# nktoan/h-edit

Hardware: AMD Instinct MI355X
Metric: edited images/sec (512^2, 50 steps, K Langevin) (higher is better)
Workload: dtype bf16

## Files before the change

h-edit_amd/build.py:

```python
#!/usr/bin/env python3
import os
import subprocess
import sys
from concurrent.futures import ThreadPoolExecutor

HERE = os.path.dirname(os.path.abspath(__file__))
SRC = os.path.join(HERE, "csrc")
OBJ = os.path.join(HERE, "build")
OUT = os.path.join(HERE, "hedit", "libhedit_hip.so")
UNITS = ["gemm.hip", "pgemm.hip", "pconv.hip", "ffn.hip", "linchain.hip", "norm.hip", "attn.hip", "attnbwd.hip", "step.hip", "grad.hip", "s2dgrad.hip", "pnet.hip", "encoder.hip", "store.hip", "unet.hip", "vae.hip", "ddpm.hip", "irse.hip", "faceparse.hip", "lpips.hip", "vit.hip", "text.hip", "clipimg.hip", "sqlpips.hip", "dino.hip", "pixmetrics.hip", "c_api.hip"]
FLAGS = ["--offload-arch=gfx950", "-O3", "-std=c++17", "-fPIC", "-ffp-contract=off", "-Wno-unused-result"]
UNIT_FLAGS = {"attn.hip": ["-fno-honor-nans"], "ffn.hip": ["-fno-honor-nans"]}


def _deps_mtime():
    hdrs = [os.path.join(SRC, f) for f in os.listdir(SRC) if f.endswith(".h")]
    hdrs.append(os.path.join(os.path.dirname(HERE), "include", "hedit.h"))
    return max(os.path.getmtime(p) for p in hdrs)


def build(force=False, verbose=True, f16=False):
    hipcc = os.environ.get("HIPCC", "/opt/rocm/bin/hipcc")
    OBJ = os.path.join(HERE, "build_f16" if f16 else "build")
    OUT = os.path.join(HERE, "hedit", "libhedit_hip_f16.so" if f16 else "libhedit_hip.so")
    FLAGS = globals()["FLAGS"] + (["-DHEDIT_STORE_F16"] if f16 else [])
    os.makedirs(OBJ, exist_ok=True)
    hm = _deps_mtime()
    jobs = []
    for u in UNITS:
        src = os.path.join(SRC, u)
        obj = os.path.join(OBJ, u.replace(".hip", ".o"))
        if force or not os.path.exists(obj) or os.path.getmtime(obj) < max(os.path.getmtime(src), hm):
            jobs.append((src, obj))

    def cc(job):
        src, obj = job
        cmd = [hipcc] + FLAGS + UNIT_FLAGS.get(os.path.basename(src), []) + ["-c", src, "-o", obj]
        r = subprocess.run(cmd, capture_output=True, text=True)
        if r.returncode != 0:
            raise RuntimeError(f"hipcc failed for {src}:\n{r.stderr[-4000:]}")
        return src

    if jobs:
        with ThreadPoolExecutor(max_workers=min(6, len(jobs))) as ex:
            for s in ex.map(cc, jobs):
                if verbose:
                    print("compiled", os.path.relpath(s, HERE))
    objs = [os.path.join(OBJ, u.replace(".hip", ".o")) for u in UNITS]
    if jobs or not os.path.exists(OUT):
        cmd = [hipcc, "--offload-arch=gfx950", "-shared", "-fPIC", "-o", OUT] + objs
        r = subprocess.run(cmd, capture_output=True, text=True)
        if r.returncode != 0:
            raise RuntimeError(f"link failed:\n{r.stderr[-4000:]}")
        if verbose:
            print("linked", os.path.relpath(OUT, HERE))
    return OUT


if __name__ == "__main__":
    build(force="--force" in sys.argv, f16="--f16" in sys.argv)
```

h-edit_amd/csrc/gemm.hip:

```cpp
#include <type_traits>

#include "common.h"
#include "gnstat.h"
#include "kernels.h"

namespace {

typedef __attribute__((ext_vector_type(4))) unsigned u32x4;
constexpr int BM0 = 128;
constexpr int BK = 64;

template <int BM, int BN, bool DEEP = false>
struct Smem {
  static constexpr int A_BYTES = BM * BK * 2;
  static constexpr int W_BYTES = BN * BK * 2;
  static constexpr int STAGE = A_BYTES + W_BYTES;
  static constexpr int STAGES = (DEEP || (BM == 256 && BN <= 160)) ? 3 : 2;
  static constexpr int EPI = BM * (BN + 8) * 2;
  static constexpr int TOTAL = STAGES * STAGE > EPI ? STAGES * STAGE : EPI;
  static constexpr int RS_W0 = 2 * A_BYTES;
  static constexpr int RS_ZERO = RS_W0 + 3 * W_BYTES;
  static constexpr int RS_TOTAL = RS_ZERO + A_BYTES + 128;
};

// ... 672 lines not shown
      float2* red = reinterpret_cast<float2*>(smem + RED_OFF);
      const int r = tid / CHUNKS, c = tid - r * CHUNKS;
      GnPiece t[2];
#pragma unroll
      for (int it = 0; it < ITER; ++it) {
        const GnPiece g = gns_piece(ov[it][0], ov[it][1], ov[it][2], ov[it][3]);
        if (gns_first<RSTEP>(it)) t[gns_slot<RSTEP>(it)] = g; else gns_add(t[gns_slot<RSTEP>(it)], g);
      }
      gns_store_t(red, gns_red_row<RSTEP>(r, 0), c, t[0]);
      gns_store_t(red, gns_red_row<RSTEP>(r, 1), c, t[1]);
      __syncthreads();
      if (tid < UNITS * 64) {
        const int u = tid >> 6, pk = tid & 63;
        const float2 v = gns_fold_unit(red, u, pk);
        if (m0 + u * GNS_UNIT < p.M)
          *reinterpret_cast<float2*>(p.gn_part + (((long)(m0 / GNS_UNIT + u) * (p.N / 2)) + n0 / 2 + pk) * 2) = v;
      }
    }
  } else {
    for (int idx = tid; idx < BM * CHUNKS * 2; idx += NT) {
      const int ml = idx / (CHUNKS * 2), h = idx - ml * (CHUNKS * 2);
      const int m = m0 + ml, n = n0 + h * 4;
      if (m >= p.M || n >= p.N) continue;
      uint2 o = *reinterpret_cast<const uint2*>(sc + ml * CS + h * 4);
      if (p.residual) {
        const uint2 r = *reinterpret_cast<const uint2*>(p.residual + (long)m * p.ldr + n);
        o.x = add2(o.x, r.x);
        o.y = add2(o.y, r.y);
      }
      *reinterpret_cast<uint2*>(p.C + (long)m * p.ldc + n) = o;
    }
  }
}

__global__ __launch_bounds__(256) void splitk_reduce_kernel(GemmParams p) {
  const long idx = (long)blockIdx.x * 256 + threadIdx.x;
  const int n4 = p.N / 4;
  const long total = (long)p.M * n4;
  if (idx >= total) return;
  const int m = (int)(idx / n4);
  const int n = (int)(idx - (long)m * n4) * 4;
  f32x4 v = {0.f, 0.f, 0.f, 0.f};
  for (int s = 0; s < p.splits; ++s)
    v += *reinterpret_cast<const f32x4*>(p.partial + ((long)s * p.M + m) * p.N + n);
  if (p.raw_f32) {
    *reinterpret_cast<f32x4*>(p.raw_f32 + (long)m * p.N + n) = v;
    return;
  }
  f32x4 b = {0.f, 0.f, 0.f, 0.f};
  if (p.bias) b = *reinterpret_cast<const f32x4*>(p.bias + n);
  v = v + b;
  uint2 o;
  o.x = pack_bf16x2(v[0], v[1]);
  o.y = pack_bf16x2(v[2], v[3]);
  if (p.residual) {
    const uint2 r = *reinterpret_cast<const uint2*>(p.residual + (long)m * p.ldr + n);
    o.x = pack_bf16x2(bf16_to_f32((bf16_t)(o.x & 0xffff)) + bf16_to_f32((bf16_t)(r.x & 0xffff)),
                      bf16_to_f32((bf16_t)(o.x >> 16)) + bf16_to_f32((bf16_t)(r.x >> 16)));
    o.y = pack_bf16x2(bf16_to_f32((bf16_t)(o.y & 0xffff)) + bf16_to_f32((bf16_t)(r.y & 0xffff)),
                      bf16_to_f32((bf16_t)(o.y >> 16)) + bf16_to_f32((bf16_t)(r.y >> 16)));
  }
  *reinterpret_cast<uint2*>(p.C + (long)m * p.ldc + n) = o;
}

__global__ __launch_bounds__(256) void splitk_reduce_gn_kernel(GemmParams p) {
  __shared__ float2 red[32 * 64];
  const int tid = threadIdx.x, r = tid >> 4, c = tid & 15;
  const int m0 = blockIdx.x * GNS_UNIT, n = blockIdx.y * 128 + c * 8;
  f32x4 b0 = {0.f, 0.f, 0.f, 0.f}, b1 = b0;
  if (p.bias) {
    b0 = *reinterpret_cast<const f32x4*>(p.bias + n);
    b1 = *reinterpret_cast<const f32x4*>(p.bias + n + 4);
  }
  auto add2 = [](uint32_t a, uint32_t b) __attribute__((always_inline)) {
    return pack_bf16x2(bf16_to_f32((bf16_t)(a & 0xffff)) + bf16_to_f32((bf16_t)(b & 0xffff)),
                       bf16_to_f32((bf16_t)(a >> 16)) + bf16_to_f32((bf16_t)(b >> 16)));
  };
  GnPiece t[2];
#pragma unroll
  for (int it = 0; it < 8; ++it) {
    const int m = m0 + r + 16 * it;
    f32x4 v0 = {0.f, 0.f, 0.f, 0.f}, v1 = v0;
    for (int s = 0; s < p.splits; ++s) {
      const float* src = p.partial + ((long)s * p.M + m) * p.N + n;
      v0 += *reinterpret_cast<const f32x4*>(src);
      v1 += *reinterpret_cast<const f32x4*>(src + 4);
    }
    v0 = v0 + b0;
    v1 = v1 + b1;
    u32x4 o = {pack_bf16x2(v0[0], v0[1]), pack_bf16x2(v0[2], v0[3]), pack_bf16x2(v1[0], v1[1]), pack_bf16x2(v1[2], v1[3])};
    if (p.residual) {
      const u32x4 rr = *reinterpret_cast<const u32x4*>(p.residual + (long)m * p.ldr + n);
      o[0] = add2(o[0], rr[0]); o[1] = add2(o[1], rr[1]); o[2] = add2(o[2], rr[2]); o[3] = add2(o[3], rr[3]);
    }
    *reinterpret_cast<u32x4*>(p.C + (long)m * p.ldc + n) = o;
    const GnPiece g = gns_piece(o[0], o[1], o[2], o[3]);
    if (gns_first<16>(it)) t[gns_slot<16>(it)] = g; else gns_add(t[gns_slot<16>(it)], g);
  }
  gns_store_t(red, gns_red_row<16>(r, 0), c, t[0]);
  gns_store_t(red, gns_red_row<16>(r, 1), c, t[1]);
  __syncthreads();
  if (tid < 64) {
    const float2 v = gns_fold_unit(red, 0, tid);
    *reinterpret_cast<float2*>(p.gn_part + ((long)blockIdx.x * (p.N / 2) + blockIdx.y * 64 + tid) * 2) = v;
  }
}

template <int BM, int BN, int MODE, bool CHUNK, bool DEEP = false>
int launch_igemm_impl(const GemmParams& p, int splits, hipStream_t st) {
  using S = Smem<BM, BN, DEEP>;
  constexpr int LDS = (MODE == 4 || MODE == 5) ? S::RS_TOTAL : S::TOTAL;
  dim3 grid(cdiv(p.M, BM) * cdiv(p.N, BN), splits);
#if HEDIT_F16
  if (p.op_bf16) {
    if (int rc = hedit_dyn_lds(reinterpret_cast<const void*>(&igemm_kernel<BM, BN, MODE, CHUNK, false, DEEP, false, true>), LDS)) return rc;
    hipLaunchKernelGGL((igemm_kernel<BM, BN, MODE, CHUNK, false, DEEP, false, true>), grid, dim3(BM * 2), LDS, st, p);
    LAUNCH_CHECK();
    return HEDIT_OK;
  }
#endif
  if constexpr (BN == 128 && MODE != 0) {
    if (p.gn_part && !p.partial) {
      if (int rc = hedit_dyn_lds(reinterpret_cast<const void*>(&igemm_kernel<BM, BN, MODE, CHUNK, false, DEEP, true>), LDS)) return rc;
      hipLaunchKernelGGL((igemm_kernel<BM, BN, MODE, CHUNK, false, DEEP, true>), grid, dim3(BM * 2), LDS, st, p);
      LAUNCH_CHECK();
      return HEDIT_OK;
    }
  }
  constexpr bool COUNTED = MODE == 4 || MODE == 5 || S::STAGES == 3;
  if constexpr (COUNTED) {
    if (hedit_test_drained()) {
      if (int rc = hedit_dyn_lds(reinterpret_cast<const void*>(&igemm_kernel<BM, BN, MODE, CHUNK, true, DEEP>), LDS)) return rc;
      hipLaunchKernelGGL((igemm_kernel<BM, BN, MODE, CHUNK, true, DEEP>), grid, dim3(BM * 2), LDS, st, p);
      LAUNCH_CHECK();
      return HEDIT_OK;
    }
  }
  if (int rc = hedit_dyn_lds(reinterpret_cast<const void*>(&igemm_kernel<BM, BN, MODE, CHUNK, false, DEEP>), LDS)) return rc;
  hipLaunchKernelGGL((igemm_kernel<BM, BN, MODE, CHUNK, false, DEEP>), grid, dim3(BM * 2), LDS, st, p);
  LAUNCH_CHECK();
  return HEDIT_OK;
}


template <int BN, int MODE>
int launch_igemm(const GemmParams& p, int splits, hipStream_t st) {
  const long tiles256 = (long)cdiv(p.M, 256) * cdiv(p.N, BN);
  const bool big = splits == 1 && (p.geglu || p.K / BK >= 16) && tiles256 >= 200;
  const bool chunk = splits == 1 && p.chunk_kt > 0 && p.chunk_kt < p.K / BK;
  if constexpr (MODE == 1) {
    if (big && splits == 1 && p.Hout == p.Hin && p.Wout == p.Win && p.Win > 0 && 256 % p.Win == 0) {
      if (!chunk) return launch_igemm_impl<256, BN, 4, false>(p, splits, st);
      if constexpr (BN == 128) return launch_igemm_impl<256, BN, 4, true>(p, splits, st);
    }
  }
  if constexpr (MODE == 3) {
    if (big && splits == 1 && p.Wout > 0 && 256 % p.Wout == 0) {
      if (!chunk) return launch_igemm_impl<256, BN, 5, false>(p, splits, st);
      if constexpr (BN == 128) return launch_igemm_impl<256, BN, 5, true>(p, splits, st);
    }
  }
  if (chunk)
    return big ? launch_igemm_impl<256, BN, MODE, true>(p, splits, st) : launch_igemm_impl<128, BN, MODE, true>(p, splits, st);
  if (big) return launch_igemm_impl<256, BN, MODE, false>(p, splits, st);
  int cus = 256;
  if (int rc = hedit_cu_count(&cus)) return rc;
  const long blocks = (long)cdiv(p.M, 128) * cdiv(p.N, BN) * splits;
  if (blocks <= cus && p.K / BK >= 3) return launch_igemm_impl<128, BN, MODE, false, true>(p, splits, st);
  return launch_igemm_impl<128, BN, MODE, false>(p, splits, st);
}

}

int gemm_pick_bn(int N);
static int pick_bn(const GemmParams& p) {
  if (p.geglu) return (p.N % 256 == 0 && (long)cdiv(p.M, 256) * (p.N / 256) >= 200) ? 256 : 128;
  return gemm_pick_bn(p.N);
}

int gemm_pick_bn(int N) {
  long w160 = (long)cdiv(N, 160) * 160, w128 = (long)cdiv(N, 128) * 128;
  return w160 <= w128 ? 160 : 128;
}

int gemm_canonical_chunk(int M_nom, int N_nom, int K) {
  const int bn = gemm_pick_bn(N_nom);
  const long tiles = (long)cdiv(M_nom, BM0) * cdiv(N_nom, bn);
  const int kt = K / BK;
  if (tiles >= 256 || kt < 24) return 0;
  int s = (int)((256 + tiles - 1) / tiles);
  int max_s = kt / 4;
  if (s > max_s) s = max_s;
  if (s > 16) s = 16;
  if (s <= 1) return 0;
  const int chunk = cdiv(kt, s);
  return chunk >= kt ? 0 : chunk;
}

int gemm_plan_splits(int M, int N, int K, int chunk_kt) {
  const int kt = K / BK;
  if (chunk_kt <= 0 || chunk_kt >= kt) return 1;
  const int s = cdiv(kt, chunk_kt);
  const long tiles = (long)cdiv(M, BM0) * cdiv(N, gemm_pick_bn(N));
  return tiles * s <= 1024 ? s : 1;
}

int gemm_pick_splits(int M, int N, int K, int force) {
  (void)M; (void)N;
  const int kt = K / BK;
  if (force <= 1) return 1;
  return force > kt ? kt : force;
}

size_t gemm_partial_bytes(int M, int N, int splits) {
  return splits > 1 ? (size_t)splits * M * N * sizeof(float) : 0;
}

static const bf16_t* zero_page_device() {
  static bf16_t* z = nullptr;
  if (!z) {
    void* ptr = nullptr;
    if (hipMalloc(&ptr, 256) != hipSuccess) return nullptr;
    if (hipMemset(ptr, 0, 256) != hipSuccess) return nullptr;
    z = reinterpret_cast<bf16_t*>(ptr);
  }
  return z;
}

int gemm_prepare() { return zero_page_device() ? HEDIT_OK : HEDIT_ERR_HIP; }

int gemm_launch(GemmParams p, int splits, float* partial_ws, hipStream_t st) {
  p.zeros = zero_page_device();
  if (!p.zeros) {
    hedit_set_error("gemm: could not allocate the zero page");
    return HEDIT_ERR_HIP;
  }
  ARG_CHECK(p.K % BK == 0, "gemm: K must be a multiple of 64");
  ARG_CHECK(p.N % 4 == 0, "gemm: N must be a multiple of 4");
  ARG_CHECK(p.mode >= 0 && p.mode <= 3, "gemm: mode");
  if (p.mode != 0) ARG_CHECK(p.Cin % BK == 0 && p.K == 9 * p.Cin, "gemm: conv needs Cin % 64 == 0 and K = 9 Cin");
  ARG_CHECK(p.ldc % 4 == 0 && (p.residual == nullptr || p.ldr % 4 == 0), "gemm: ldc/ldr alignment");
  {
    const double a_b = p.mode == 0 ? (double)p.M * p.lda * 2.0
                                   : (double)(p.M / ((long)p.Hout * p.Wout)) * p.Hin * p.Win * p.Cin * 2.0;
    const double w_b = (double)p.N * p.K * 2.0;
    ARG_CHECK(a_b < 2040.0 * 1048576.0 && w_b < 2040.0 * 1048576.0, "gemm: operand larger than 2 GiB");
    p.a_bytes = (unsigned)a_b;
    p.w_bytes = (unsigned)w_b;
  }
  const int kt = p.K / BK;
  if (splits < 1) splits = 1;
  if (splits > kt) splits = kt;
  if (p.chunk_kt < 0 || p.chunk_kt >= kt) p.chunk_kt = 0;
  if (splits > 1) {
    p.kt_per_split = p.chunk_kt > 0 ? p.chunk_kt : cdiv(kt, splits);
    p.splits = cdiv(kt, p.kt_per_split);
    ARG_CHECK(p.chunk_kt == 0 || p.splits == splits, "gemm: split count does not match the canonical chunking");
  } else {
    p.splits = 1;
    p.kt_per_split = kt;
  }
  splits = p.splits;
  if (p.raw_f32 && splits == 1) {
    ARG_CHECK(!p.geglu, "gemm: raw fp32 output excludes the GEGLU epilogue");
    p.partial = p.raw_f32;
  } else if (splits > 1) {
    ARG_CHECK(!p.geglu, "gemm: split-K excludes the GEGLU epilogue");
    ARG_CHECK(partial_ws != nullptr, "gemm: split-K needs a partial workspace");
    p.partial = partial_ws;
  } else {
    p.partial = nullptr;
  }
  ARG_CHECK(!p.op_bf16 || (p.raw_f32 && !p.geglu && !p.gn_part), "gemm: bfloat16-by-contract operands come with the raw fp32 output");
  if (p.gn_part) {
    ARG_CHECK(p.mode != 0 && !p.geglu && !p.raw_f32 && !p.ln_out, "gemm: pair statistics come with the bf16 tile of a convolution");
    ARG_CHECK(p.M % GNS_UNIT == 0 && p.N % 128 == 0 && gemm_pick_bn(p.N) == 128, "gemm: pair statistics need M % 128 == 0 and the 128-column tile");
    ARG_CHECK(p.ldc % 8 == 0 && (p.residual == nullptr || p.ldr % 8 == 0), "gemm: pair statistics need 16-byte rows");
  }
  int bn = pick_bn(p);
  if (splits == 1 && p.chunk_kt > 0 && p.mode == 3) bn = 128;
  if (splits == 1 && p.chunk_kt > 0 && p.mode == 1 && p.Hout == p.Hin && p.Wout == p.Win && p.Win > 0 && 256 % p.Win == 0 &&
      p.N % 128 == 0 && (long)cdiv(p.M, 256) * (p.N / 128) >= 512)
    bn = 128;
  if (p.geglu) {
    ARG_CHECK(p.N % 32 == 0 && p.mode == 0 && p.residual == nullptr && p.ldc % 8 == 0, "gemm: geglu epilogue needs N % 32 == 0, linear mode, no residual");
    ARG_CHECK(splits == 1 && p.chunk_kt == 0, "gemm: the geglu epilogue takes no K-chunking");
  }
  {
    const double a_bytes = (double)p.M * (p.mode == 0 ? p.K : p.Cin);
    const double w_bytes = (double)p.N * p.K;
    p.n_fastest = a_bytes >= w_bytes ? 1 : 0;
  }
  if (pgemm_supported(p, splits, bn)) return pgemm_launch(p, bn, st);
  if (pconv_supported(p, splits, bn)) return pconv_launch(p, bn, st);
  int rc;
#define DISPATCH(BNV)                                                     \
  switch (p.mode) {                                                       \
    case 0: rc = launch_igemm<BNV, 0>(p, splits, st); break;              \
    case 1: rc = launch_igemm<BNV, 1>(p, splits, st); break;              \
    case 2: rc = launch_igemm<BNV, 2>(p, splits, st); break;              \
    default: rc = launch_igemm<BNV, 3>(p, splits, st); break;             \
  }
  if (bn == 256) {
    rc = launch_igemm_impl<256, 256, 0, false>(p, 1, st);
  } else if (bn == 160) { DISPATCH(160) } else { DISPATCH(128) }
#undef DISPATCH
  if (rc != HEDIT_OK) return rc;
  if (splits > 1) {
    if (p.ln_out && p.ln_done && !p.raw_f32 && p.ldc == p.N && splitk_reduce_ln_supported(p.N)) {
      *p.ln_done = 1;
      return splitk_reduce_ln_launch(p.partial, p.splits, p.bias, p.residual, p.ldr, p.C, p.ln_out, p.ln_gamma, p.ln_beta, p.M, p.N,
                                     p.ln_eps, st);
    }
    if (p.gn_part) {
      hipLaunchKernelGGL(splitk_reduce_gn_kernel, dim3(p.M / GNS_UNIT, p.N / 128), dim3(256), 0, st, p);
      LAUNCH_CHECK();
      return HEDIT_OK;
    }
    long total = (long)p.M * (p.N / 4);
    hipLaunchKernelGGL(splitk_reduce_kernel, dim3(cdiv(total, 256)), dim3(256), 0, st, p);
    LAUNCH_CHECK();
  }
  return HEDIT_OK;
}
```

h-edit_amd/csrc/kernels.h:

```cpp
#pragma once
#include "common.h"

struct GemmParams {
  const bf16_t* A;
  const bf16_t* W;
  int M, N, K;
  int lda;
  int mode;
  int Hin, Win, Cin, Hout, Wout;
  const float* bias;
  const bf16_t* residual;
  int ldr;
  bf16_t* C;
  int ldc;
  float* partial;
  int splits, kt_per_split;
  int n_fastest;
  const bf16_t* zeros;
  unsigned a_bytes, w_bytes;
  int geglu;
  int asym;
  float* raw_f32;
  int chunk_kt;
  const float *ln_gamma, *ln_beta;
  bf16_t* ln_out;
  float ln_eps;
  int* ln_done;
  float* gn_part;
  int op_bf16;
};
#ifndef GEMM_NOMINAL_BATCH
#define GEMM_NOMINAL_BATCH 4
#endif
int gemm_prepare();
int gemm_pick_bn(int N);
int gemm_pick_splits(int M, int N, int K, int force);
int gemm_canonical_chunk(int M_nom, int N_nom, int K);
int gemm_plan_splits(int M, int N, int K, int chunk_kt);
size_t gemm_partial_bytes(int M, int N, int splits);
int gemm_launch(GemmParams p, int splits, float* partial_ws, hipStream_t st);
bool pgemm_supported(const GemmParams& p, int splits, int bn);
int pgemm_launch(const GemmParams& p, int bn, hipStream_t st);
bool pconv_supported(const GemmParams& p, int splits, int bn);
int pconv_launch(const GemmParams& p, int bn, hipStream_t st);

struct FfnParams {
  const bf16_t* x; long ldx;
  const float* gamma; const float* beta; float eps;
  const bf16_t* stream;
  const float* bias1p;
  const float* bias2;
  bf16_t* out; long ldo;
  int M, C;
  const bf16_t* a; long lda;
  const bf16_t* r2; long ldr2;
  const float* bias_pre; const float* bias_post;
};
struct LinChainParams {
  const bf16_t* a; long lda;
  const bf16_t* r1; long ldr1;
  const float* bias_pre;
  const float* gamma; const float* beta; float eps;
  const bf16_t* stream;
  bf16_t* out_mid; long ldmid;
  bf16_t* out; long ldo;
  int M, C;
  const float* gn_ss; int rows_per_image;
  bf16_t* out_q; long ldq; bf16_t* out_k; long ldk;
};
int lin_chain_launch(const LinChainParams& c, hipStream_t st);
int lin_chain_launch_sched(const LinChainParams& c, int sched, hipStream_t st);
size_t lin_chain_stream_bytes(int layers);
int lin_chain_pack_launch(const float* w, int layer, float scale, int layers, bf16_t* stream, hipStream_t st);
int ffn_fused_channels();
size_t ffn_stream_bytes(int pre, int post);
size_t ffn_bias_bytes();
int ffn_pack_launch(const float* w, int which, int pre, int post, bf16_t* stream, hipStream_t st);
int ffn_pack_bias_launch(const float* b1, float* out, hipStream_t st);
int ffn_fused_launch(const FfnParams& f, hipStream_t st);

#define HEDIT_MAXW 77
#define HEDIT_WPAD 96
#define HEDIT_CTXP 80

size_t groupnorm_ws_bytes(int B, int HW, int C);
int groupnorm_launch(const bf16_t* x, bf16_t* y, const float* gamma, const float* beta, int B,
                     int HW, int C, int G, float eps, int silu, float* ws, hipStream_t st,
                     float* stats = nullptr);
bool groupnorm_from_parts_supported(int HW, int C, int G);
size_t groupnorm_from_parts_ws_bytes(int B);
int groupnorm_from_parts_launch(const bf16_t* x, bf16_t* y, const float* gamma, const float* beta, int B, int HW, int C, int G,
                                float eps, int silu, const float* part_a, int ca, const float* part_b, int cb, float* ws,
                                hipStream_t st);
int groupnorm_affine_launch(const bf16_t* x, const float* gamma, const float* beta, int B, int HW, int C, int G, float eps,
                            float* ws, hipStream_t st, const float** ss_out);
int layernorm_launch(const bf16_t* x, bf16_t* y, const float* gamma, const float* beta, long rows,
                     int C, float eps, hipStream_t st);
bool splitk_reduce_ln_supported(int C);
int splitk_reduce_ln_launch(const float* partial, int splits, const float* bias, const bf16_t* residual, int ldr, bf16_t* out,
                            bf16_t* y, const float* gamma, const float* beta, long rows, int C, float eps, hipStream_t st);
int geglu_launch(const bf16_t* x, bf16_t* y, long rows, int inner, hipStream_t st);
#define HEDIT_ROWMAP_MAX 512
struct RowMap { uint16_t src[HEDIT_ROWMAP_MAX]; };
int concat_launch(const bf16_t* a, int ca, const bf16_t* b, int cb, bf16_t* y, long rows, hipStream_t st,
                  const RowMap* b_map = nullptr, int rows_per_image = 0);
int gather_rows_launch(const void* const* src, void* const* dst, int n, int B, long row_bytes, const RowMap& map, hipStream_t st);
int f32_to_bf16_launch(const float* x, bf16_t* y, long n, hipStream_t st);
int ctx_pad_launch(const float* x, bf16_t* y, int B, int dim, hipStream_t st);
int gemv_launch(const bf16_t* W, const float* x, const float* b0, const float* b1, float* out,
                int N, int K, int silu, hipStream_t st);
int copy_rows_launch(bf16_t* x, const int* src, int B, long row_elems, hipStream_t st);
int timestep_embed_launch(float t, float* out, int dim, hipStream_t st);
int timestep_embed_ddpm_launch(float t, float* out, int dim, hipStream_t st);
int conv_in_launch(const float* x, const float* w, const float* bias, bf16_t* y, int B, int Cin,
                   int H, int W, int Cout, hipStream_t st);
int conv_out_launch(const bf16_t* x, const bf16_t* w, const float* bias, float* y, int B, int H,
                    int W, int C, int Cout, hipStream_t st);
int rows_to_nchw_launch(const float* src, const float* bias, float* dst, int B, long HW, int ld, int Cout, hipStream_t st);
int softmax_rows_launch(const float* s, bf16_t* p, long rows, int N, float scale, hipStream_t st);
int softmax_blockdiag_launch(const float* s, bf16_t* p, long rows, int T, int ld, float scale, hipStream_t st);
int mix1x1_nchw_launch(const float* x, const float* w, const float* bias, float* y, int B, int Cin, int Cout, long HW,
                       float pre_scale, hipStream_t st);
int quant_mean_launch(const bf16_t* h, const float* w, const float* bias, float* y, int B, long HW, int Cm, int Cout, hipStream_t st);
int pack_linear_launch(const float* w, bf16_t* out, long n, float scale, hipStream_t st);
int pack_conv3x3_launch(const float* w_oihw, bf16_t* out, int O, int I, hipStream_t st);
int pack_geglu_rows_launch(const float* w, bf16_t* out_bf16, float* out_f32, int rows, int K, hipStream_t st);

size_t groupnorm_bwd_ws_bytes(int B, int HW, int C);
int groupnorm_bwd_launch(const bf16_t* x, const bf16_t* dy, const bf16_t* add, bf16_t* dx, const float* gamma,
                         const float* beta, const float* stats, int B, int HW, int C, int G, int silu, float* ws,
                         hipStream_t st, bool any_width = false);
int softmax_bwd_launch(const bf16_t* p, const float* dp, bf16_t* ds, long rows, int N, float scale, hipStream_t st);
int transpose_bf16_launch(const bf16_t* src, bf16_t* dst, int R, int C, hipStream_t st);
int sum2x2_launch(const bf16_t* du, bf16_t* dx, int B, int H, int W, int C, hipStream_t st);
int pack_conv3x3_dgrad_launch(const float* w_oihw, bf16_t* out, int O, int I, hipStream_t st);
int pack_linear_t_launch(const float* w, bf16_t* out, int O, int I, hipStream_t st, float scale = 1.f, long ldo = 0);
int flip_oihw_launch(const float* w, float* out, int O, int I, int k, hipStream_t st);
int layernorm_bwd_launch(const bf16_t* x, const bf16_t* dy, const bf16_t* add, bf16_t* dx, const float* gamma, long rows, int C,
                         float eps, hipStream_t st);
int geglu_bwd_launch(const bf16_t* x, const bf16_t* dy, bf16_t* dx, long rows, int inner, hipStream_t st);

int conv3x3_s2_dgrad_launch(const bf16_t* dy, const bf16_t* wt, bf16_t* dx, int B, int Hin, int Win, int O, int I, hipStream_t st);
int pack_conv3x3_s2_dgrad_launch(const float* w_oihw, bf16_t* out, int O, int I, hipStream_t st);
int conv3x3_s2_dgrad_pad1_launch(const bf16_t* dy, const bf16_t* wt, bf16_t* dx, int B, int Hin, int Win, int O, int I, hipStream_t st);
int slice_add_launch(const bf16_t* src, int ld, int off, int c, bf16_t* dst, long rows, int accumulate, hipStream_t st);

struct SelfAttnParams {
  const bf16_t* q; int ldq;
  const bf16_t* k; int ldk;
  const bf16_t* vt; long ldvt;
  bf16_t* out; int ldo;
  int B, N, heads, d;
  const int* qk_src;
  const int* kv_src;
  int test_flags;
};
int self_attn_launch(const SelfAttnParams& p, hipStream_t st);

struct CrossAttnParams {
  const bf16_t* q; int ldq;
  const bf16_t* k; int ldk;
  const bf16_t* vt; long ldvt;
  bf16_t* out; int ldo;
  int B, N, heads, d;
  int n_pairs;
  const int* pair_src;
  const int* pair_tar;
  const bf16_t* mixT;
  const float* bvec;
  float* store;
  const int* singles;
  int n_single;
};
int cross_attn_launch(const CrossAttnParams& p, hipStream_t st);

struct AttnProbsParams {
  const bf16_t* q; int ldq;
  const bf16_t* k; int ldk;
  const bf16_t* vt; long ldvt;
  float* probs;
  bf16_t* out; int ldo;
  int B, N, M, kstride, heads, d;
  const int *pair_src, *pair_tar, *qk_src;
};
int attn_probs_launch(const AttnProbsParams& p, hipStream_t st);
int attn_self_store_launch(const AttnProbsParams& p, hipStream_t st);
int attn_apply_launch(const AttnProbsParams& p, hipStream_t st);

struct AttnBwdParams {
  const bf16_t* q; int ldq;
  const bf16_t* k; int ldk;
  const bf16_t* v; int ldv;
  const bf16_t* o; int ldo;
  const bf16_t* dout; int lddo;
  bf16_t* dq; int lddq;
  bf16_t* dk; bf16_t* dv; int lddkv;
  float* stats;
  int B, N, M, kstride, heads, d;
};
size_t attn_bwd_ws_bytes(int B, int N, int heads);
int attn_bwd_launch(const AttnBwdParams& p, hipStream_t st);
int attn_bwd_ctx_chunk(int N);
size_t attn_bwd_ctx_kv_ws_bytes(int B, int N, int heads, int d);
int attn_bwd_ctx_kv_launch(const AttnBwdParams& p, float* part, hipStream_t st);

struct StepCoef {
  float sqrt_ab_t, sqrt_1m_ab_t;
  float sqrt_ab_prev;
  float dir_coef;
  float noise_coef;
  float w_src, w_hat, w_tar;
  float coeff;
  float w_rec;
};
int step_base_launch(const float* eps, const float* xt, const float* z, float* x_prev, int n_img,
                     int elems, int eps_rows_per_img, StepCoef c, hipStream_t st);
int step_pair_launch(const float* e_u, const float* e_c, const float* xt, const float* z, float* x_next, int n_img, int elems,
                     int n_kinds, const StepCoef* c, hipStream_t st);
int step_invert_launch(const float* e_u, const float* e_c, const float* xt, float* x_prev, float* z_out, int n_img,
                       int elems, StepCoef c, hipStream_t st);
int step_update_launch(const float* e_u_src, const float* e_c_src, const float* e_u_tar,
                       const float* e_c_tar, long stride_img, const float* x_k, const float* x_base,
                       float* x_out, int n_img, int elems, int k_gt0, StepCoef c, hipStream_t st);
int step_tweedie_launch(const float* e_u_tar, const float* e_c_tar, long stride_img, const float* x, float* z0,
                        int n_img, int elems, float w_tar, float sqrt_ab, float sqrt_1m_ab, float inv_scale, hipStream_t st);
int step_style_launch(const float* e_u_src, const float* e_c_src, const float* e_u_tar, const float* e_c_tar,
                      long stride_img, const float* x, const float* g_z, float* x_out, int n_img, int elems, float w_hat,
                      float w_tar, float chain, float weight, hipStream_t st);
int step_ef_seed_launch(const float* g_z, float* d_eps, int n_img, int elems, float w_tar, float c, hipStream_t st);
int step_ef_style_launch(const float* e_u, const float* e_c, long stride_img, const float* dx, const float* g_z,
                         const float* x_prev, float* x_out, int n_img, int elems, float a, float weight, hipStream_t st);
int axis_mix_launch(const float* in, float* out, const int* idx, const float* val, int nnz, long outer, int n_in, int n_out, int inner,
                    hipStream_t st);
int local_blend_launch(const float* const* maps, int n_maps, int heads, const float* alpha_layers, const float* alpha_sub,
                       const int* enabled, float* xt, int n_img, int C, int H, int W, float th, float th_sub, hipStream_t st);

enum { P_COPY = 0, P_AFFINE = 1, P_PRELU = 2, P_PRELU_GRAD = 3, P_RELU = 4, P_RELU_GRAD = 5, P_QGELU = 6, P_QGELU_GRAD = 7,
       P_AFFINE_RELU = 8,
       P_GELU = 9 };
struct Split3Params {
  const float* x; int ldx;
  const float* z;
  const float* p; const float* q;
  int pq_img;
  int op;
  bf16_t* out; int Kp, Cs, C;
  int geo;
  int B, H, W;
  int worder;
};
int split3_launch(const Split3Params& s, long rows_out, hipStream_t st);
int pack_split3_w_launch(const float* w, const float* scale, bf16_t* out, int O, int I, int k, int dgrad, int Cs, int Kp,
                         int rows_out, int perm_hw, int perm_c, hipStream_t st);
int bn_affine_launch(const float* g, const float* b, const float* m, const float* v, float eps, float* p, float* q, int C, int rep,
                     hipStream_t st);
int bn_fold_bias_launch(const float* bias, const float* g, const float* b, const float* m, const float* v, float eps, float* p, float* q,
                        int C, hipStream_t st);
int act_launch(const float* x, const float* p, const float* q, float* y, long total, int C, int op, hipStream_t st);
int se_nslab(int HW);
int se_pool_launch(const float* u, float* part, int B, int HW, int C, hipStream_t st);
int se_fc_launch(const float* part, const float* bias, const float* w1, const float* w2, float* hbuf, float* sbuf, int B, int HW, int C,
                 int R, hipStream_t st);
int se_combine_launch(const float* u, const float* bias, const float* s, const float* sc, const float* sc_bias, const float* X, int stride,
                      float* Y, int B, int Ho, int Wo, int C, hipStream_t st);
int se_bwd_reduce_launch(const float* dY, const float* u, const float* bias, float* part, int B, int HW, int C, hipStream_t st);
int se_fc_bwd_launch(const float* part, const float* sbuf, const float* hbuf, const float* w1, const float* w2, float* rbuf, int B, int C,
                     int R, int HW, hipStream_t st);
int unit_bwd_combine_launch(const float* dxa, const float* p, const float* dsc, int stride, float* dX, int B, int H, int W, int C,
                            hipStream_t st);
int scale_cols_launch(const float* x, const float* p, float* y, long total, int n, hipStream_t st);
int face_pool_launch(const float* img, float* out, int B, hipStream_t st);
int face_pool_bwd_launch(const float* g, int ldg, float* dimg, int B, hipStream_t st);
int cos_head_launch(const float* raw, const float* bias, const float* ref, int ref_stride, float* feat, float* loss, float* df, int B, int D,
                    float scale, hipStream_t st);
int lpips_prep_launch(const float* img, float* out, const float* shift3, const float* scale3, int B, int H, int W, hipStream_t st);
int lpips_prep_bwd_launch(const float* g, int ldg, float* dimg, const float* scale3, int B, int H, int W, hipStream_t st);
int maxpool2_launch(const float* z, float* zp, uint8_t* idx, int B, int H, int W, int C, hipStream_t st);
int maxpool2_bwd_launch(const float* gp, const uint8_t* idx, const float* add, float* G, int B, int H, int W, int C, hipStream_t st);
int lpips_head_launch(const float* z, const float* bias, const float* src, long src_img_stride, const float* w, float* fn_out, float* dpix,
                      float* dF, int B, int HW, int C, float gscale, hipStream_t st);
int lpips_reduce_launch(const float* dpix, float* acc, int B, int HW, int first, hipStream_t st);

int enc_patchify_launch(const float* img, float* X, int B, int R, int p, int bwd, hipStream_t st);
int enc_tokens_launch(const float* E, const float* cbias, const float* cls, const float* pos, float* T, int B, int L, int W, hipStream_t st);
int enc_gather_rows_launch(const float* T, const int32_t* idx, float* R, int B, int L, int W, hipStream_t st);
int enc_ln_launch(const float* x, const float* g, const float* b, float* y, float* stats, long rows, int W, float eps, hipStream_t st);
int enc_add_bias_res_launch(const float* raw, const float* bias, const float* res, float* out, long total, int W, hipStream_t st);
```

Baseline: 2.675.

## Add persistent pipelined GEMM kernel with fused GEGLU epilogue

Adds a new persistent kernel for the 256x256 GEGLU GEMM path. It launches one block per CU, walks tiles in an XCD-aware order, and double-buffers K stages with direct buffer-to-LDS loads. The next tile's first loads are prefetched while the current tile's epilogue runs. The GEGLU epilogue goes through per-wave LDS scratch so global stores are coalesced 16-byte writes. The path is used only when there are at least twice as many tiles as CUs; otherwise the existing igemm is kept. This adds code complexity and LDS pressure.

```diff
diff --git a/h-edit_amd/build.py b/h-edit_amd/build.py
--- a/h-edit_amd/build.py
+++ b/h-edit_amd/build.py
@@ -8,7 +8,7 @@
 SRC = os.path.join(HERE, "csrc")
 OBJ = os.path.join(HERE, "build")
 OUT = os.path.join(HERE, "hedit", "libhedit_hip.so")
-UNITS = ["gemm.hip", "pgemm.hip", "pconv.hip", "ffn.hip", "linchain.hip", "norm.hip", "attn.hip", "attnbwd.hip", "step.hip", "grad.hip", "s2dgrad.hip", "pnet.hip", "encoder.hip", "store.hip", "unet.hip", "vae.hip", "ddpm.hip", "irse.hip", "faceparse.hip", "lpips.hip", "vit.hip", "text.hip", "clipimg.hip", "sqlpips.hip", "dino.hip", "pixmetrics.hip", "c_api.hip"]
+UNITS = ["gemm.hip", "pgemm.hip", "pgeglu.hip", "pconv.hip", "ffn.hip", "linchain.hip", "norm.hip", "attn.hip", "attnbwd.hip", "step.hip", "grad.hip", "s2dgrad.hip", "pnet.hip", "encoder.hip", "store.hip", "unet.hip", "vae.hip", "ddpm.hip", "irse.hip", "faceparse.hip", "lpips.hip", "vit.hip", "text.hip", "clipimg.hip", "sqlpips.hip", "dino.hip", "pixmetrics.hip", "c_api.hip"]
 FLAGS = ["--offload-arch=gfx950", "-O3", "-std=c++17", "-fPIC", "-ffp-contract=off", "-Wno-unused-result"]
 UNIT_FLAGS = {"attn.hip": ["-fno-honor-nans"], "ffn.hip": ["-fno-honor-nans"]}
 
diff --git a/h-edit_amd/csrc/gemm.hip b/h-edit_amd/csrc/gemm.hip
--- a/h-edit_amd/csrc/gemm.hip
+++ b/h-edit_amd/csrc/gemm.hip
@@ -998,7 +998,7 @@
     default: rc = launch_igemm<BNV, 3>(p, splits, st); break;             \
   }
   if (bn == 256) {
-    rc = launch_igemm_impl<256, 256, 0, false>(p, 1, st);
+    rc = pgeglu_supported(p) ? pgeglu_launch(p, st) : launch_igemm_impl<256, 256, 0, false>(p, 1, st);
   } else if (bn == 160) { DISPATCH(160) } else { DISPATCH(128) }
 #undef DISPATCH
   if (rc != HEDIT_OK) return rc;
diff --git a/h-edit_amd/csrc/kernels.h b/h-edit_amd/csrc/kernels.h
--- a/h-edit_amd/csrc/kernels.h
+++ b/h-edit_amd/csrc/kernels.h
@@ -41,6 +41,8 @@
 int gemm_launch(GemmParams p, int splits, float* partial_ws, hipStream_t st);
 bool pgemm_supported(const GemmParams& p, int splits, int bn);
 int pgemm_launch(const GemmParams& p, int bn, hipStream_t st);
+bool pgeglu_supported(const GemmParams& p);
+int pgeglu_launch(const GemmParams& p, hipStream_t st);
 bool pconv_supported(const GemmParams& p, int splits, int bn);
 int pconv_launch(const GemmParams& p, int bn, hipStream_t st);
 
diff --git a/h-edit_amd/csrc/pgeglu.hip b/h-edit_amd/csrc/pgeglu.hip
--- /dev/null
+++ b/h-edit_amd/csrc/pgeglu.hip
@@ -0,0 +1,264 @@
+#include "common.h"
+#include "kernels.h"
+
+namespace {
+
+typedef __attribute__((ext_vector_type(4))) unsigned u32x4;
+constexpr int BK = 64;
+constexpr int BM = 256;
+constexpr int BN = 256;
+constexpr int NT = 512;
+constexpr unsigned OOB = 0x80000000u;
+#ifndef PGG_ABL
+#define PGG_ABL 0
+#endif
+constexpr int ABL = PGG_ABL;
+
+struct GS {
+  static constexpr int A_BYTES = BM * BK * 2;
+  static constexpr int W_BYTES = BN * BK * 2;
+  static constexpr int STAGE = A_BYTES + W_BYTES;
+  static constexpr int ON = BN / 2;
+  static constexpr int SCR_STRIDE = (ON / 2) * 2 + 16;
+  static constexpr int SCR0 = 2 * STAGE;
+  static constexpr int SCR_BYTES = 16 * SCR_STRIDE;
+  static constexpr int BIAS0 = SCR0 + 8 * SCR_BYTES;
+  static constexpr int BIAS_SLOT = BN * 2;
+  static constexpr int TOTAL = BIAS0 + 8 * BIAS_SLOT;
+  static_assert(SCR_BYTES % 16 == 0 && BIAS0 % 16 == 0, "16-byte pieces");
+  static_assert(TOTAL <= 160 * 1024, "stages + scratch must fit the LDS");
+};
+
+struct TileWalk {
+  int first, step, count;
+  __device__ TileWalk(int nb, int grid, int bid) {
+    const int xcd = bid & 7, cidx = bid >> 3;
+    const int q8 = nb >> 3, r8 = nb & 7;
+    const int X0 = xcd < r8 ? xcd * (q8 + 1) : r8 * (q8 + 1) + (xcd - r8) * q8;
+    const int XN = q8 + (xcd < r8 ? 1 : 0);
+    step = (grid - xcd + 7) >> 3;
+    first = X0 + cidx;
+    count = cidx < XN ? (XN - cidx + step - 1) / step : 0;
+  }
+};
+
+__global__ __launch_bounds__(NT, 2) void pgeglu_kernel(GemmParams p) {
+  extern __shared__ __attribute__((aligned(16))) char smem[];
+  const unsigned lds_base = (unsigned)(uintptr_t)(__attribute__((address_space(3))) char*)smem;
+  using S = GS;
+  constexpr int NI = BN / 32, MI = 4;
+  constexpr int A_CH = 4, W_CH = 4;
+  constexpr int PCH = S::ON / 2 / 8;
+  constexpr int NQ = 16 * PCH / 64;
+  static_assert(NQ == 2, "a 16-row pass of a wave is two pieces per lane");
+
+  const int tid = threadIdx.x;
+  const int lane = tid & 63;
+  const int wave = __builtin_amdgcn_readfirstlane(tid >> 6);
+  const int wm = wave >> 1, wn = wave & 1;
+  const int fr = lane & 15, fq = lane >> 4;
+
+  const int tiles_m = (p.M + BM - 1) / BM;
+  const int tiles_n = p.N / BN;
+  const TileWalk walk(tiles_m * tiles_n, gridDim.x, blockIdx.x);
+  const int T = walk.count;
+  if (T == 0) return;
+  const int nk = p.K / BK;
+
+  const unsigned lda2 = (unsigned)p.lda * 2u, ldc2 = (unsigned)p.ldc * 2u, K2 = (unsigned)p.K * 2u;
+  auto tile_mn = [&](int k, int& m0, int& n0) __attribute__((always_inline)) {
+    const int v = walk.first + k * walk.step;
+    const int tm = p.n_fastest ? v / tiles_n : v % tiles_m;
+    const int tn = p.n_fastest ? v % tiles_n : v / tiles_m;
+    m0 = tm * BM;
+    n0 = tn * BN;
+  };
+  const int drow = wave * 32 + (lane >> 3);
+  const unsigned dchunk = (unsigned)(((lane & 7) ^ (lane >> 3)) * 16);
+  const unsigned a_lane = (unsigned)drow * lda2 + dchunk, w_lane = (unsigned)drow * K2 + dchunk;
+#if defined(__HIP_DEVICE_COMPILE__)
+  const __amdgpu_buffer_rsrc_t rs_a = __builtin_amdgcn_make_buffer_rsrc(const_cast<bf16_t*>(p.A), (short)0, (int)p.a_bytes, 0x00020000);
+  const __amdgpu_buffer_rsrc_t rs_w = __builtin_amdgcn_make_buffer_rsrc(const_cast<bf16_t*>(p.W), (short)0, (int)p.w_bytes, 0x00020000);
+  const __amdgpu_buffer_rsrc_t rs_c = __builtin_amdgcn_make_buffer_rsrc(p.C, (short)0, (int)((unsigned)p.M * ldc2), 0x00020000);
+  const __amdgpu_buffer_rsrc_t rs_b =
+      __builtin_amdgcn_make_buffer_rsrc(const_cast<float*>(p.bias), (short)0, p.bias ? p.N * 4 : 0, 0x00020000);
+#endif
+  auto fire = [&](int buf, int kt, int m0, int n0) __attribute__((always_inline)) {
+#if defined(__HIP_DEVICE_COMPILE__)
+    char* sa = smem + buf * S::STAGE;
+    char* sw = sa + S::A_BYTES;
+    const int left = p.M - m0;
+#pragma unroll
+    for (int i = 0; i < A_CH; ++i) {
+      const unsigned off = drow + i * 8 < left ? a_lane + (unsigned)(m0 + i * 8) * lda2 : OOB;
+      __builtin_amdgcn_raw_ptr_buffer_load_lds(rs_a, (__attribute__((address_space(3))) void*)(sa + (wave * A_CH + i) * 1024), 16, off, kt * 128, 0, 0);
+    }
+#pragma unroll
+    for (int i = 0; i < W_CH; ++i)
+      __builtin_amdgcn_raw_ptr_buffer_load_lds(rs_w, (__attribute__((address_space(3))) void*)(sw + (wave * W_CH + i) * 1024), 16,
+                                               w_lane + (unsigned)(n0 + i * 8) * K2, kt * 128, 0, 0);
+#else
+    (void)buf; (void)kt; (void)m0; (void)n0;
+#endif
+  };
+  auto bias_fire = [&](int n0) __attribute__((always_inline)) {
+#if defined(__HIP_DEVICE_COMPILE__)
+    if (lane < BN / 8)
+      __builtin_amdgcn_raw_ptr_buffer_load_lds(rs_b, (__attribute__((address_space(3))) void*)(smem + S::BIAS0 + wave * S::BIAS_SLOT), 16,
+                                               (unsigned)(n0 + wn * (BN / 2) + lane * 4) * 4u, 0, 0, 0);
+#else
+    (void)n0;
+#endif
+  };
+
+  const int rd_x = ((fq ^ (fr & 7)) << 4);
+  const int a_rd = (wm * 64 + fr) * 128 + rd_x;
+  const int w_rd = (wn * (BN / 2) + fr) * 128 + rd_x;
+  bf16x8 xa[MI], wa[NI], xb[MI], wb[NI];
+  auto read_frags = [&](int buf, int ks, bf16x8 (&xf)[MI], bf16x8 (&wf)[NI]) __attribute__((always_inline)) {
+    const char* pa = smem + buf * S::STAGE + (a_rd ^ (ks << 6));
+    const char* pw = smem + buf * S::STAGE + S::A_BYTES + (w_rd ^ (ks << 6));
+#pragma unroll
+    for (int i = 0; i < MI; ++i) xf[i] = *reinterpret_cast<const bf16x8*>(pa + i * 2048);
+#pragma unroll
+    for (int j = 0; j < NI; ++j) wf[j] = *reinterpret_cast<const bf16x8*>(pw + j * 2048);
+  };
+  f32x4 acc[MI][NI];
+  auto mfmas = [&](const bf16x8 (&xf)[MI], const bf16x8 (&wf)[NI]) __attribute__((always_inline)) {
+#pragma unroll
+    for (int i = 0; i < MI; ++i)
+#pragma unroll
+      for (int j = 0; j < NI; ++j) acc[i][j] = MFMA_16x16x32_ST(wf[j], xf[i], acc[i][j], 0, 0, 0);
+  };
+  auto mfma_group = [&](const bf16x8 (&xf)[MI], const bf16x8 (&wf)[NI]) __attribute__((always_inline)) {
+    __builtin_amdgcn_s_setprio(1);
+    mfmas(xf, wf);
+    __builtin_amdgcn_s_setprio(0);
+  };
+
+  const int scr = (int)lds_base + S::SCR0 + wave * S::SCR_BYTES;
+  const unsigned scr_wr = (unsigned)(scr + fr * S::SCR_STRIDE + fq * 8);
+  const int pr = lane / PCH, pc = lane - pr * PCH;
+  const unsigned scr_rd = (unsigned)(scr + pr * S::SCR_STRIDE + pc * 16);
+  const int c_row = wm * 64 + pr;
+  const unsigned c_lane = (unsigned)c_row * ldc2 + (unsigned)(wn * (S::ON / 2) + pc * 8) * 2u;
+
+  int m0, n0;
+  tile_mn(0, m0, n0);
+  bias_fire(n0);
+  fire(0, 0, m0, n0);
+  asm volatile("s_waitcnt vmcnt(0)\n\ts_barrier" ::: "memory");
+  if (nk > 1) fire(1, 1, m0, n0);
+  read_frags(0, 0, xa, wa);
+
+  for (int t = 0; t < T; ++t) {
+#pragma unroll
+    for (int i = 0; i < MI; ++i)
+#pragma unroll
+      for (int j = 0; j < NI; ++j) acc[i][j] = (f32x4){0.f, 0.f, 0.f, 0.f};
+    int i = 0;
+    for (; i + 2 < nk; ++i) {
+      const int cur = i & 1;
+      read_frags(cur, 1, xb, wb);
+      __builtin_amdgcn_s_setprio(1);
+      mfmas(xa, wa);
+      __builtin_amdgcn_s_setprio(0);
+      asm volatile("s_waitcnt vmcnt(0) lgkmcnt(0)\n\ts_barrier" ::: "memory");
+      __builtin_amdgcn_s_setprio(1);
+      read_frags(cur ^ 1, 0, xa, wa);
+      fire(cur, i + 2, m0, n0);
+      mfmas(xb, wb);
+#pragma unroll
+      for (int r = 0; r < MI * NI / 2; ++r) {
+        __builtin_amdgcn_sched_group_barrier(0x008, 2, 0);
+        if (r < (MI + NI + 1) / 2) {
+          __builtin_amdgcn_sched_group_barrier(0x100, 2, 0);
+        } else {
+          __builtin_amdgcn_sched_group_barrier(0x004, 2, 0);
+          __builtin_amdgcn_sched_group_barrier(0x020, 2, 0);
+        }
+      }
+      __builtin_amdgcn_s_setprio(0);
+    }
+    if (i + 1 < nk) {
+      const int cur = i & 1;
+      read_frags(cur, 1, xb, wb);
+      mfma_group(xa, wa);
+      asm volatile("s_waitcnt vmcnt(0) lgkmcnt(0)\n\ts_barrier" ::: "memory");
+      read_frags(cur ^ 1, 0, xa, wa);
+      mfma_group(xb, wb);
+      ++i;
+    }
+    read_frags(i & 1, 1, xb, wb);
+    mfma_group(xa, wa);
+    asm volatile("s_waitcnt vmcnt(0) lgkmcnt(0)\n\ts_barrier" ::: "memory");
+    const bool more = t + 1 < T;
+    int m0n = 0, n0n = 0;
+    if (more) {
+      tile_mn(t + 1, m0n, n0n);
+      fire(0, 0, m0n, n0n);
+      if (nk > 1) fire(1, 1, m0n, n0n);
+    }
+    mfma_group(xb, wb);
+
+    f32x4 bv[NI];
+#pragma unroll
+    for (int j = 0; j < NI; ++j)
+      bv[j] = *reinterpret_cast<const f32x4*>(smem + S::BIAS0 + wave * S::BIAS_SLOT + (j * 16 + fq * 4) * 4);
+#pragma unroll
+    for (int ps = 0; ps < ((ABL & 8) ? 0 : MI); ++ps) {
+#pragma unroll
+      for (int j = 0; j < NI; j += 2) {
+        const f32x4 v = acc[ps][j] + bv[j], g = acc[ps][j + 1] + bv[j + 1];
+        uint2 o;
+        const f32x2 r0 = mul_gelu2((f32x2){v[0], v[1]}, (f32x2){g[0], g[1]});
+        const f32x2 r1 = mul_gelu2((f32x2){v[2], v[3]}, (f32x2){g[2], g[3]});
+        o.x = pack_bf16x2(r0[0], r0[1]);
+        o.y = pack_bf16x2(r1[0], r1[1]);
+        asm volatile("ds_write_b64 %0, %1 offset:%2" ::"v"(scr_wr), "v"(__builtin_bit_cast(unsigned long long, o)), "n"((j / 2) * 32) : "memory");
+      }
+      u32x4 ov[NQ];
+#pragma unroll
+      for (int q = 0; q < NQ; ++q)
+        asm volatile("ds_read_b128 %0, %1 offset:%2" : "=v"(ov[q]) : "v"(scr_rd), "n"(q * 8 * S::SCR_STRIDE) : "memory");
+      asm volatile("s_waitcnt lgkmcnt(0)" : "+v"(ov[0]), "+v"(ov[1])::"memory");
+#pragma unroll
+      for (int q = 0; q < NQ; ++q) {
+        const int mt = ps * 16 + q * 8;
+#if defined(__HIP_DEVICE_COMPILE__)
+        __builtin_amdgcn_raw_buffer_store_b128(ov[q], rs_c, c_row + mt < p.M - m0 && !(ABL & 1) ? c_lane + (unsigned)(m0 + mt) * ldc2 + (unsigned)n0 : OOB, 0, 0);
+#else
+        (void)mt;
+#endif
+      }
+    }
+    if (!more) break;
+    asm volatile("s_waitcnt lgkmcnt(0)" ::: "memory");
+    bias_fire(n0n);
+    m0 = m0n;
+    n0 = n0n;
+    asm volatile("s_waitcnt vmcnt(0)\n\ts_barrier" ::: "memory");
+    read_frags(0, 0, xa, wa);
+  }
+}
+
+}
+
+bool pgeglu_supported(const GemmParams& p) {
+  if (hedit_test_flags() & 8) return false;
+  if (!p.geglu || p.N % BN != 0 || p.mode != 0 || p.partial || p.raw_f32 || p.residual) return false;
+  if ((double)p.M * p.ldc * 2.0 >= 2040.0 * 1048576.0) return false;
+  int cus = 256;
+  if (hedit_cu_count(&cus)) return false;
+  const long tiles = (long)cdiv(p.M, BM) * (p.N / BN);
+  return tiles >= 2L * cus;
+}
+
+int pgeglu_launch(const GemmParams& p, hipStream_t st) {
+  int cus = 256;
+  if (int rc = hedit_cu_count(&cus)) return rc;
+  if (int rc = hedit_dyn_lds(reinterpret_cast<const void*>(&pgeglu_kernel), GS::TOTAL)) return rc;
+  hipLaunchKernelGGL(pgeglu_kernel, dim3(cus), dim3(NT), GS::TOTAL, st, p);
+  LAUNCH_CHECK();
+  return HEDIT_OK;
+}
```

New measurement: 2.683, median of 6. No clear change (+0.3%).
